# huggingface/parler-tts

Measured on NVIDIA H100. Metric: audio codec tokens/sec (all codebooks), higher is better.
Workload: dtype bf16

## Files before the change

### parler_tts_b200/csrc/attn_core.cuh

```cuda
#pragma once
#include "common.cuh"
#include "kernels.h"

namespace ptts {

constexpr int ATT_THREADS = 128;
constexpr int ATT_WARPS = 4;
constexpr int HD = PTTS_HEAD_DIM;

template <typename Sync>
__device__ __forceinline__ float block_reduce(float v, float* sh, bool is_max, int tid, Sync sync) {
  const int warp = tid >> 5, lane = tid & 31;
  v = is_max ? warp_max(v) : warp_sum(v);
  sync();
  if (lane == 0) sh[warp] = v;
  sync();
  float r = sh[0];
#pragma unroll
  for (int w = 1; w < ATT_WARPS; w++) r = is_max ? fmaxf(r, sh[w]) : r + sh[w];
  return r;
}

template <typename T>
__device__ __forceinline__ float rope_elem(float x, float x_pair, int d, const T* cos_row, const T* sin_row) {
// ... 11 lines not shown
  float* red = sm + HD;
  float* sh = red + ATT_WARPS * HD;
  float* sc = sh + 8;
  const int warp = tid >> 5, lane = tid & 31;
  const int rep = p.nh / p.nkv;
  int past = p.past_len;
  if (p.past_from_ctrl) past = p.prefix + p.ctrl->cur_len - 1;

  T* kc = reinterpret_cast<T*>(p.kcache) + (size_t)b * p.kv_b_stride + (size_t)kvh * p.kv_h_stride;
  T* vc = reinterpret_cast<T*>(p.vcache) + (size_t)b * p.kv_b_stride + (size_t)kvh * p.kv_h_stride;

  if (!p.cross) {
    const int d = tid & 63;
    const bool is_v = tid >= 64;
    for (int j = 0; j < p.q_len && j < q_hi; j++) {
      const size_t r = (size_t)b * p.q_len + j;
      const int pos = past + j;
      if (!is_v) {
        const T* src = reinterpret_cast<const T*>(p.knew) + r * p.ldkv + p.k_col0 + kvh * HD;
        float x = DT<T>::to_f(src[d]);
        if (p.rope) {
          const float xp = DT<T>::to_f(src[d < HD / 2 ? d + HD / 2 : d - HD / 2]);
          x = rope_elem<T>(x, xp, d, rope_cos + (size_t)pos * HD, rope_sin + (size_t)pos * HD);
        }
        kc[(size_t)pos * p.kv_t_stride + kv_swz(pos, d)] = DT<T>::from_f(x);
      } else {
        const T* src = reinterpret_cast<const T*>(p.vnew) + r * p.ldkv + p.v_col0 + kvh * HD;
        vc[(size_t)pos * p.kv_t_stride + kv_swz(pos, d)] = src[d];
      }
    }
    sync();
  }

  const int grp = lane >> 3;
  const int d0 = (lane & 7) * 8;
  const int kslot = warp * 4 + grp;
  const int* km = p.key_mask ? p.key_mask + (size_t)b * p.mask_ld : nullptr;

  for (int j = q_lo; j < p.q_len && j < q_hi; j++) {
    const size_t r = (size_t)b * p.q_len + j;
    const int pos = past + j;
    const int T_keys = p.cross ? p.kv_len : pos + 1;
    for (int rr = 0; rr < rep; rr++) {
      const int h = kvh * rep + rr;
      sync();
      if (tid < HD) {
        const T* src = reinterpret_cast<const T*>(p.q) + r * p.ldq + p.q_col0 + h * HD;
        float x = DT<T>::to_f(src[tid]);
        if (p.rope) {
          const float xp = DT<T>::to_f(src[tid < HD / 2 ? tid + HD / 2 : tid - HD / 2]);
          x = rope_elem<T>(x, xp, tid, rope_cos + (size_t)pos * HD, rope_sin + (size_t)pos * HD);
        }
        qs[tid] = x;
      }
      sync();
      float qv[8];
#pragma unroll
      for (int e = 0; e < 8; e++) qv[e] = qs[d0 + e];

      float lmax = -INFINITY;
      for (int t0 = 0; t0 < T_keys; t0 += 64) {
        float kv[4][8];
        bool ok[4];
#pragma unroll
        for (int u = 0; u < 4; u++) {
          const int t = t0 + u * 16 + kslot;
          ok[u] = t < T_keys;
          if (ok[u]) load8(kc + (size_t)t * p.kv_t_stride + kv_swz(t, d0), kv[u]);
        }
#pragma unroll
        for (int u = 0; u < 4; u++) {
          const int t = t0 + u * 16 + kslot;
          float s = 0.f;
          if (ok[u]) {
#pragma unroll
            for (int e = 0; e < 8; e++) s = fmaf(qv[e], kv[u][e], s);
          }
          s += __shfl_xor_sync(0xffffffffu, s, 1);
          s += __shfl_xor_sync(0xffffffffu, s, 2);
          s += __shfl_xor_sync(0xffffffffu, s, 4);
          if (ok[u] && (lane & 7) == 0) {
            s *= p.scale;
            if (km != nullptr && t < p.mask_len && km[t] == 0) s = -INFINITY;
            sc[t] = s;
            lmax = fmaxf(lmax, s);
          }
        }
      }
      const float m = block_reduce(lmax, sh, true, tid, sync);
      float lsum = 0.f;
      for (int t = tid; t < T_keys; t += ATT_THREADS) {
        const float e = (m == -INFINITY) ? 1.0f : expf(sc[t] - m);
        sc[t] = e;
        lsum += e;
      }
      const float l = block_reduce(lsum, sh, false, tid, sync);
      float acc[8];
#pragma unroll
      for (int e = 0; e < 8; e++) acc[e] = 0.f;
      for (int t0 = 0; t0 < T_keys; t0 += 64) {
        float vv[4][8];
        float pw[4];
#pragma unroll
        for (int u = 0; u < 4; u++) {
          const int t = t0 + u * 16 + kslot;
          pw[u] = 0.f;
          if (t < T_keys) {
            load8(vc + (size_t)t * p.kv_t_stride + kv_swz(t, d0), vv[u]);
            pw[u] = DT<T>::rnd(sc[t]);
          } else {
#pragma unroll
            for (int e = 0; e < 8; e++) vv[u][e] = 0.f;
          }
        }
#pragma unroll
        for (int u = 0; u < 4; u++)
#pragma unroll
          for (int e = 0; e < 8; e++) acc[e] = fmaf(pw[u], vv[u][e], acc[e]);
      }
#pragma unroll
      for (int e = 0; e < 8; e++) {
        acc[e] += __shfl_xor_sync(0xffffffffu, acc[e], 8);
        acc[e] += __shfl_xor_sync(0xffffffffu, acc[e], 16);
      }
      if (lane < 8) {
#pragma unroll
        for (int e = 0; e < 8; e++) red[warp * HD + d0 + e] = acc[e];
      }
      sync();
      if (tid < HD) {
        float o = red[tid] + red[HD + tid] + red[2 * HD + tid] + red[3 * HD + tid];
        o = o / l;
        reinterpret_cast<T*>(p.out)[r * p.ldo + h * HD + tid] = DT<T>::from_f(o);
      }
    }
  }
}

}

namespace ptts {

__device__ __forceinline__ uint32_t att_smem_u32(const void* p) { return (uint32_t)__cvta_generic_to_shared(p); }

template <typename T> struct AttChunk { static constexpr int CH = 32; };
template <> struct AttChunk<float> { static constexpr int CH = 16; };

template <typename T, int CH = AttChunk<T>::CH>
__host__ __device__ constexpr int attn_decode_smem_per_warp() {
  return 2 * 2 * CH * HD * (int)sizeof(T) + (3 * HD) * (int)sizeof(float);
}

template <typename T, int CH = AttChunk<T>::CH>
__device__ __forceinline__ void attention_decode_item_warp(const AttnArgs& p, int b, int kvh, int pos, unsigned char* sm_warp, uint64_t* bars,
                                                           int lane, uint32_t& parity, int part = 0, int nparts = 1, float* xch = nullptr,
                                                           int pair_bar = 0) {
  constexpr int STAGE_ELEMS = CH * HD;
  T* kst = reinterpret_cast<T*>(sm_warp);
  T* vst = kst + 2 * STAGE_ELEMS;
  float* qs = reinterpret_cast<float*>(vst + 2 * STAGE_ELEMS);
  float* kn = qs + HD;
  float* vn = kn + HD;
  const T* __restrict__ rope_cos = reinterpret_cast<const T*>(p.rope_cos) + (size_t)pos * HD;
  const T* __restrict__ rope_sin = reinterpret_cast<const T*>(p.rope_sin) + (size_t)pos * HD;
  const int rep = p.nh / p.nkv;
  T* kc = reinterpret_cast<T*>(p.kcache) + (size_t)b * p.kv_b_stride + (size_t)kvh * p.kv_h_stride;
  T* vc = reinterpret_cast<T*>(p.vcache) + (size_t)b * p.kv_b_stride + (size_t)kvh * p.kv_h_stride;
  const int lo = lane, hi = lane + HD / 2;
  const int n_cached = p.cross ? p.kv_len : pos;
  const int n_chunks_all = (n_cached + CH - 1) / CH;
  const int n_chunks = (n_chunks_all > part) ? (n_chunks_all - part + nparts - 1) / nparts : 0;

  auto issue = [&](int i) {
    const int st = i & 1;
    const int t0 = (part + nparts * i) * CH;
    const int n = (n_cached - t0 < CH) ? (n_cached - t0) : CH;
    const uint32_t bar = att_smem_u32(&bars[st]);
    if (lane == 0) asm volatile("mbarrier.arrive.expect_tx.shared::cta.b64 _, [%0], %1;" ::"r"(bar), "r"((uint32_t)(2 * n * HD * sizeof(T))) : "memory");
    __syncwarp();
    if (lane < 2) {
      const T* src = (lane == 0 ? kc : vc) + (size_t)t0 * HD;
      T* dst = (lane == 0 ? kst : vst) + st * STAGE_ELEMS;
      asm volatile("cp.async.bulk.shared::cluster.global.mbarrier::complete_tx::bytes [%0], [%1], %2, [%3];"
                   ::"r"(att_smem_u32(dst)), "l"(src), "r"((uint32_t)(n * HD * sizeof(T))), "r"(bar) : "memory");
    }
  };
  auto wait_stage = [&](int st) {
    const uint32_t bar = att_smem_u32(&bars[st]);
    const uint32_t par = (parity >> st) & 1u;
    uint32_t ok, spins = 0;
    do {
      asm volatile("{\n.reg .pred p;\nmbarrier.try_wait.parity.shared::cta.b64 p, [%1], %2;\nselp.u32 %0, 1, 0, p;\n}" : "=r"(ok) : "r"(bar), "r"(par) : "memory");
      if (!ok && ++spins > (1u << 16)) { if (lane == 0) printf("ptts: attention KV mbarrier timeout (cta %d b %d kvh %d stage %d cross %d n_cached %d chunks %d par %u)\n", (int)blockIdx.x, b, kvh, st, p.cross, n_cached, n_chunks, parity); __trap(); }
    } while (!ok);
    parity ^= (1u << st);
  };

  __syncwarp();
  asm volatile("fence.proxy.async.shared::cta;" ::: "memory");
  if (n_chunks > 0) issue(0);
  if (n_chunks > 1) issue(1);

  const T* q_first = reinterpret_cast<const T*>(p.q) + (size_t)b * p.ldq + p.q_col0 + (size_t)(kvh * rep) * HD;
  const float qf0 = DT<T>::to_f(q_first[lo]), qf1 = DT<T>::to_f(q_first[hi]);
  if (!p.cross && part == 0) {
    const T* ksrc = reinterpret_cast<const T*>(p.knew) + (size_t)b * p.ldkv + p.k_col0 + kvh * HD;
    const T* vsrc = reinterpret_cast<const T*>(p.vnew) + (size_t)b * p.ldkv + p.v_col0 + kvh * HD;
    float x0 = DT<T>::to_f(ksrc[lo]), x1 = DT<T>::to_f(ksrc[hi]);
    if (p.rope) {
      const float y0 = rope_elem<T>(x0, x1, lo, rope_cos, rope_sin);
      const float y1 = rope_elem<T>(x1, x0, hi, rope_cos, rope_sin);
      x0 = y0; x1 = y1;
    }
    const T v0 = vsrc[lo], v1 = vsrc[hi];
    kc[(size_t)pos * p.kv_t_stride + kv_swz(pos, lo)] = DT<T>::from_f(x0);
    kc[(size_t)pos * p.kv_t_stride + kv_swz(pos, hi)] = DT<T>::from_f(x1);
    vc[(size_t)pos * p.kv_t_stride + kv_swz(pos, lo)] = v0;
    vc[(size_t)pos * p.kv_t_stride + kv_swz(pos, hi)] = v1;
    kn[lo] = DT<T>::rnd(x0); kn[hi] = DT<T>::rnd(x1);
    vn[lo] = DT<T>::to_f(v0); vn[hi] = DT<T>::to_f(v1);
  }
  const int grp = lane >> 3, d0 = (lane & 7) * 8;
  const int* km = p.key_mask ? p.key_mask + (size_t)b * p.mask_ld : nullptr;

  for (int rr = 0; rr < rep; rr++) {
    const int h = kvh * rep + rr;
    {
      const T* qsrc = reinterpret_cast<const T*>(p.q) + (size_t)b * p.ldq + p.q_col0 + h * HD;
      float x0 = (rr == 0) ? qf0 : DT<T>::to_f(qsrc[lo]), x1 = (rr == 0) ? qf1 : DT<T>::to_f(qsrc[hi]);
      if (p.rope) {
        const float y0 = rope_elem<T>(x0, x1, lo, rope_cos, rope_sin);
        const float y1 = rope_elem<T>(x1, x0, hi, rope_cos, rope_sin);
        x0 = y0; x1 = y1;
      }
      __syncwarp();
      qs[lo] = x0; qs[hi] = x1;
      __syncwarp();
    }
    float qv[8];
#pragma unroll
    for (int e = 0; e < 8; e++) qv[e] = qs[d0 + e];
    float m_run = -INFINITY, l_run = 0.f;
    float acc[8];
#pragma unroll
    for (int e = 0; e < 8; e++) acc[e] = 0.f;

    auto process = [&](const T* kb, const T* vb, uint32_t mword, int n) {
      constexpr int PER = CH / 4;
      float sloc[PER];
#pragma unroll
      for (int u = 0; u < PER; u++) {
        const int r = u * 4 + grp, rc = r < n ? r : n - 1;
        float kf[8];
        load8(kb + rc * HD + kv_swz(rc, d0), kf);
        float s = 0.f;
#pragma unroll
        for (int e = 0; e < 8; e++) s = fmaf(qv[e], kf[e], s);
        sloc[u] = s;
      }
#pragma unroll
      for (int u = 0; u < PER; u++) sloc[u] += __shfl_xor_sync(0xffffffffu, sloc[u], 1);
#pragma unroll
      for (int u = 0; u < PER; u++) sloc[u] += __shfl_xor_sync(0xffffffffu, sloc[u], 2);
#pragma unroll
      for (int u = 0; u < PER; u++) sloc[u] += __shfl_xor_sync(0xffffffffu, sloc[u], 4);
      float cmax = -INFINITY;
#pragma unroll
      for (int u = 0; u < PER; u++) {
        const int r = u * 4 + grp;
        sloc[u] = (r < n && ((mword >> r) & 1u)) ? sloc[u] * p.scale : -INFINITY;
        cmax = fmaxf(cmax, sloc[u]);
      }
      cmax = warp_max(cmax);
      const float m_new = fmaxf(m_run, cmax);
      if (m_new == -INFINITY) return;
      const float corr = (m_run == -INFINITY) ? 0.f : expf(m_run - m_new);
      l_run *= corr;
#pragma unroll
      for (int e = 0; e < 8; e++) acc[e] *= corr;
      float lsum = 0.f;
#pragma unroll
      for (int u = 0; u < PER; u++) {
        const int r = u * 4 + grp, rc = r < n ? r : n - 1;
        const float pe = expf(sloc[u] - m_new);
        lsum += pe;
        const float pw = DT<T>::rnd(pe);
        float vf[8];
        load8(vb + rc * HD + kv_swz(rc, d0), vf);
#pragma unroll
        for (int e = 0; e < 8; e++) acc[e] = fmaf(pw, vf[e], acc[e]);
      }
      lsum += __shfl_xor_sync(0xffffffffu, lsum, 8);
      lsum += __shfl_xor_sync(0xffffffffu, lsum, 16);
      l_run += lsum;
      m_run = m_new;
    };
    auto mask_bits = [&](int t0) -> int {
      const int t = t0 + lane;
      return (km != nullptr && lane < CH && t < p.mask_len && t < n_cached) ? km[t] : 1;
    };

    if (rr > 0) {
      __syncwarp();
      asm volatile("fence.proxy.async.shared::cta;" ::: "memory");
      if (n_chunks > 0) issue(0);
      if (n_chunks > 1) issue(1);
    }
    for (int c = 0; c < n_chunks; c++) {
      const int st = c & 1;
      const int t0 = (part + nparts * c) * CH;
      const int n = (n_cached - t0 < CH) ? (n_cached - t0) : CH;
      const int mk = mask_bits(t0);
      wait_stage(st);
      process(kst + st * STAGE_ELEMS, vst + st * STAGE_ELEMS, __ballot_sync(0xffffffffu, mk != 0), n);
      if (c + 2 < n_chunks) {
        __syncwarp();
        asm volatile("fence.proxy.async.shared::cta;" ::: "memory");
        issue(c + 2);
      }
    }
    if (!p.cross && part == 0) {
      __syncwarp();
      float s = 0.f;
      if (grp == 0) {
#pragma unroll
        for (int e = 0; e < 8; e++) s = fmaf(qv[e], kn[d0 + e], s);
      }
      s += __shfl_xor_sync(0xffffffffu, s, 1);
      s += __shfl_xor_sync(0xffffffffu, s, 2);
      s += __shfl_xor_sync(0xffffffffu, s, 4);
      s = __shfl_sync(0xffffffffu, s, 0) * p.scale;
      if (km != nullptr && pos < p.mask_len && km[pos] == 0) s = -INFINITY;
      const float m_new = fmaxf(m_run, s);
      if (m_new != -INFINITY) {
        const float corr = (m_run == -INFINITY) ? 0.f : expf(m_run - m_new);
        const float pe = (s == -INFINITY) ? 0.f : expf(s - m_new);
        const float pw = DT<T>::rnd(pe);
        l_run = l_run * corr + pe;
#pragma unroll
        for (int e = 0; e < 8; e++) acc[e] = acc[e] * corr + ((grp == 0) ? pw * vn[d0 + e] : 0.f);
        m_run = m_new;
      }
    }
#pragma unroll
    for (int e = 0; e < 8; e++) {
      acc[e] += __shfl_xor_sync(0xffffffffu, acc[e], 8);
      acc[e] += __shfl_xor_sync(0xffffffffu, acc[e], 16);
    }
    if (nparts == 2) {
      if (part == 1) {
        if (lane < 8) {
#pragma unroll
          for (int e = 0; e < 8; e++) xch[d0 + e] = acc[e];
        }
        if (lane == 0) { xch[HD] = m_run; xch[HD + 1] = l_run; }
      }
      asm volatile("bar.sync %0, 64;" ::"r"(pair_bar) : "memory");
      if (part == 0) {
        const float m1 = xch[HD], l1 = xch[HD + 1];
        const float mm = fmaxf(m_run, m1);
        const float c0 = (m_run == -INFINITY) ? 0.f : expf(m_run - mm);
        const float c1 = (m1 == -INFINITY) ? 0.f : expf(m1 - mm);
        l_run = l_run * c0 + l1 * c1;
        if (lane < 8) {
#pragma unroll
          for (int e = 0; e < 8; e++) acc[e] = acc[e] * c0 + xch[d0 + e] * c1;
        }
      }
      asm volatile("bar.sync %0, 64;" ::"r"(pair_bar) : "memory");
    }
    if (lane < 8 && part == 0) {
      float o[8];
      const float inv = (l_run > 0.f) ? 1.0f / l_run : 0.f;
#pragma unroll
      for (int e = 0; e < 8; e++) o[e] = acc[e] * inv;
      store8(reinterpret_cast<T*>(p.out) + (size_t)b * p.ldo + h * HD + d0, o);
    }
  }
}

__device__ __forceinline__ void att_ldsm4(uint32_t (&r)[4], uint32_t addr) {
  asm volatile("ldmatrix.sync.aligned.m8n8.x4.shared.b16 {%0,%1,%2,%3}, [%4];" : "=r"(r[0]), "=r"(r[1]), "=r"(r[2]), "=r"(r[3]) : "r"(addr));
}
__device__ __forceinline__ void att_ldsm4_t(uint32_t (&r)[4], uint32_t addr) {
  asm volatile("ldmatrix.sync.aligned.m8n8.x4.trans.shared.b16 {%0,%1,%2,%3}, [%4];" : "=r"(r[0]), "=r"(r[1]), "=r"(r[2]), "=r"(r[3]) : "r"(addr));
}
__device__ __forceinline__ void att_mma(float (&d)[4], uint32_t a0, uint32_t a1, uint32_t a2, uint32_t a3, uint32_t b0, uint32_t b1) {
  asm volatile("mma.sync.aligned.m16n8k16.row.col.f32.bf16.bf16.f32 {%0,%1,%2,%3}, {%4,%5,%6,%7}, {%8,%9}, {%0,%1,%2,%3};"
               : "+f"(d[0]), "+f"(d[1]), "+f"(d[2]), "+f"(d[3]) : "r"(a0), "r"(a1), "r"(a2), "r"(a3), "r"(b0), "r"(b1));
}
__device__ __forceinline__ uint32_t att_pack(float lo, float hi) {
  const __nv_bfloat162 v = __floats2bfloat162_rn(lo, hi);
  return *reinterpret_cast<const uint32_t*>(&v);
}

__device__ __forceinline__ float att_ex2(float x) {
  float y;
  asm("ex2.approx.ftz.f32 %0, %1;" : "=f"(y) : "f"(x));
  return y;
}

__device__ __forceinline__ void att_bulk_kv(uint32_t dst, const void* src, uint32_t bytes, uint32_t bar, bool stream) {
  if (stream) {
    uint64_t pol;
    asm volatile("createpolicy.fractional.L2::evict_first.b64 %0, 1.0;" : "=l"(pol));
    asm volatile("cp.async.bulk.shared::cluster.global.mbarrier::complete_tx::bytes.L2::cache_hint [%0], [%1], %2, [%3], %4;"
                 ::"r"(dst), "l"(src), "r"(bytes), "r"(bar), "l"(pol) : "memory");
  } else {
    asm volatile("cp.async.bulk.shared::cluster.global.mbarrier::complete_tx::bytes [%0], [%1], %2, [%3];"
                 ::"r"(dst), "l"(src), "r"(bytes), "r"(bar) : "memory");
  }
}

constexpr int ATT_TC_CH = 32;
constexpr int ATT_TC_STAGE_BYTES = 2 * ATT_TC_CH * HD * 2;

struct TcItem {
  const bf16* q;
  const bf16* knew;
  const bf16* vnew;
  bf16* kc;
  bf16* vc;
  const int* km;
  int mask_len;
  int n_cached;
  int pos;
  int cross;
  int rope;
  const bf16* rope_cos;
  const bf16* rope_sin;
  float scale;
  bf16* out;
};

__device__ __forceinline__ void attention_tc_issue_first(const TcItem& p, unsigned char* ring0, uint64_t* bars, int lane,
                                                         int part, int nparts, bool stream = false) {
  constexpr int CH = ATT_TC_CH;
  const int n_cached = p.n_cached;
  const int t0 = part * CH;
  if (t0 >= n_cached) return;
  const int n = (n_cached - t0 < CH) ? (n_cached - t0) : CH;
  const bf16* kc = p.kc;
  const bf16* vc = p.vc;
  __syncwarp();
  const uint32_t bar = att_smem_u32(&bars[0]);
  if (lane == 0) asm volatile("mbarrier.arrive.expect_tx.shared::cta.b64 _, [%0], %1;" ::"r"(bar), "r"((uint32_t)(2 * n * HD * 2)) : "memory");
  __syncwarp();
  if (lane < 2) {
    const bf16* src = (lane == 0 ? kc : vc) + (size_t)t0 * HD;
    bf16* dst = reinterpret_cast<bf16*>(ring0) + (lane == 0 ? 0 : CH * HD);
    att_bulk_kv(att_smem_u32(dst), src, (uint32_t)(n * HD * 2), bar, stream);
  }
}

__device__ __forceinline__ void attention_decode_item_warp_tc(const TcItem& p, unsigned char* ring0, unsigned char* ring1, float* fbuf,
                                                              uint64_t* bars, int lane, uint32_t& parity, int part, int nparts, float* xch, int pair_bar,
                                                              long long* prof = nullptr, bool pre_issued = false, bool stream = false) {
  constexpr int CH = ATT_TC_CH;
  constexpr int NTS = CH / 8;
  constexpr int KPV = CH / 16;
  float* qs = fbuf;
  float* kn = qs + HD;
  float* vn = kn + HD;
  const int pos = p.pos;
  const bf16* __restrict__ rope_cos = p.rope ? p.rope_cos + (size_t)pos * HD : nullptr;
  const bf16* __restrict__ rope_sin = p.rope ? p.rope_sin + (size_t)pos * HD : nullptr;
  bf16* kc = p.kc;
// ... 228 lines not shown
```

### parler_tts_b200/csrc/step2.cu

```cuda
#include "attn_core.cuh"
#include "common.cuh"
#include "kernels.h"
#include "ln_stats.cuh"
#include "sample_core.cuh"
#include "step.h"
#include <type_traits>

#include <cstdlib>

namespace ptts {
namespace cl {

constexpr int C = 2;
constexpr int V = 8;
constexpr int THREADS = 256;
constexpr int ROWS = 32;
constexpr int HROWS = 8;
constexpr int ATT_SMEM = attn_decode_smem_per_warp<bf16>();
constexpr int PROF_STRIDE = 16;
constexpr int QMAX = 6;
constexpr int OFF_STATS = 256, OFF_PART = 512, OFF_RES = 2560, OFF_CVEC = 3584;
constexpr int HDR = 5632;
constexpr int WB_BYTES = 65536;
constexpr int R_OFF = HDR + 2 * WB_BYTES;
constexpr int R_BYTES = 92160;
constexpr int R_PASS0 = 65536;
constexpr int QKV_OFF = R_BYTES - 2048;
constexpr int SMEM_BYTES = R_OFF + R_BYTES;
static_assert(SMEM_BYTES + 1024 <= 227 * 1024, "cluster step kernel shared memory");
static_assert(ROWS * (1024 / 2 + 8) * 2 <= V * (256 + ROWS * 34 * 4) && 2 * V * (256 + ROWS * 34 * 4) <= R_BYTES, "fc1 plan");
static_assert(2 * V * C * (32 + 4 * 96 * 4) <= R_PASS0 && R_PASS0 + V * QMAX * 32 * 16 <= QKV_OFF, "QKV plan");
static_assert(5 * ATT_SMEM <= QKV_OFF && 3 * ATT_SMEM <= WB_BYTES && 16384 + 4 * 128 * 4 <= WB_BYTES, "attention plan");
static_assert(ROWS * (4096 / 4 + 8) * 2 + V * (256 + ROWS * 8 * 4) <= R_BYTES, "fc2 plan");

__device__ __forceinline__ uint32_t s32(const void* p) { return (uint32_t)__cvta_generic_to_shared(p); }
__device__ __forceinline__ void mbar_init(uint64_t* bar, uint32_t count) { asm volatile("mbarrier.init.shared::cta.b64 [%0], %1;" ::"r"(s32(bar)), "r"(count)); }
__device__ __forceinline__ void mbar_expect_tx(uint64_t* bar, uint32_t bytes) {
  asm volatile("mbarrier.arrive.expect_tx.shared::cta.b64 _, [%0], %1;" ::"r"(s32(bar)), "r"(bytes) : "memory");
}
__device__ __forceinline__ void mbar_wait(uint64_t* bar, uint32_t parity, int what) {
  uint32_t ok, spins = 0;
  do {
    asm volatile("{\n.reg .pred p;\nmbarrier.try_wait.parity.acquire.cluster.shared::cta.b64 p, [%1], %2;\nselp.u32 %0, 1, 0, p;\n}"
                 : "=r"(ok) : "r"(s32(bar)), "r"(parity) : "memory");
    if (!ok && ++spins > (1u << 22)) { printf("ptts: cluster step mbarrier timeout (cta %d, barrier kind %d)\n", (int)blockIdx.x, what); __trap(); }
  } while (!ok);
}
__device__ __forceinline__ void bulk_g2s(void* dst_smem, const void* src, uint32_t bytes, uint64_t* bar) {
  asm volatile("cp.async.bulk.shared::cluster.global.mbarrier::complete_tx::bytes [%0], [%1], %2, [%3];"
               ::"r"(s32(dst_smem)), "l"(src), "r"(bytes), "r"(s32(bar)) : "memory");
}
__device__ __forceinline__ uint64_t l2_evict_first_policy() {
  uint64_t pol;
  asm volatile("createpolicy.fractional.L2::evict_first.b64 %0, 1.0;" : "=l"(pol));
  return pol;
}
__device__ __forceinline__ void bulk_g2s_stream(void* dst_smem, const void* src, uint32_t bytes, uint64_t* bar) {
  asm volatile("cp.async.bulk.shared::cluster.global.mbarrier::complete_tx::bytes.L2::cache_hint [%0], [%1], %2, [%3], %4;"
               ::"r"(s32(dst_smem)), "l"(src), "r"(bytes), "r"(s32(bar)), "l"(l2_evict_first_policy()) : "memory");
}
__device__ __forceinline__ void bulk_s2peer(uint32_t dst_cluster_addr, const void* src_smem, uint32_t bytes, uint32_t bar_cluster_addr) {
  asm volatile("cp.async.bulk.shared::cluster.shared::cta.mbarrier::complete_tx::bytes [%0], [%1], %2, [%3];"
               ::"r"(dst_cluster_addr), "r"(s32(src_smem)), "r"(bytes), "r"(bar_cluster_addr) : "memory");
}
__device__ __forceinline__ uint32_t mapa(uint32_t addr, uint32_t rank) { uint32_t r; asm volatile("mapa.shared::cluster.u32 %0, %1, %2;" : "=r"(r) : "r"(addr), "r"(rank)); return r; }
__device__ __forceinline__ uint32_t cluster_rank() { uint32_t r; asm volatile("mov.u32 %0, %%cluster_ctarank;" : "=r"(r)); return r; }
__device__ __forceinline__ void cluster_arrive() { asm volatile("barrier.cluster.arrive.release.aligned;" ::: "memory"); }
__device__ __forceinline__ void cluster_wait() { asm volatile("barrier.cluster.wait.acquire.aligned;" ::: "memory"); }
__device__ __forceinline__ void cluster_arrive_reuse(bool release) {
  if (release) asm volatile("barrier.cluster.arrive.release.aligned;" ::: "memory");
  else asm volatile("barrier.cluster.arrive.relaxed.aligned;" ::: "memory");
}
__device__ __forceinline__ void fence_proxy_async_smem() { asm volatile("fence.proxy.async.shared::cta;" ::: "memory"); }
__device__ __forceinline__ void l2_prefetch(const void* p, uint32_t bytes, bool on = true) {
  if (!on) return;
  const char* c = reinterpret_cast<const char*>(p);
  while (bytes > 0) {
    const uint32_t n = bytes > 32768u ? 32768u : bytes;
    asm volatile("cp.async.bulk.prefetch.L2.global [%0], %1;" ::"l"(c), "r"(n) : "memory");
    c += n;
    bytes -= n;
  }
}
__device__ __forceinline__ unsigned ld_relaxed(const unsigned* p) { unsigned v; asm volatile("ld.relaxed.gpu.global.u32 %0, [%1];" : "=r"(v) : "l"(p) : "memory"); return v; }
__device__ __forceinline__ void red_release_add(unsigned* p, unsigned v) { asm volatile("red.release.gpu.global.add.u32 [%0], %1;" ::"l"(p), "r"(v) : "memory"); }
__device__ __forceinline__ void ldsm4(uint32_t (&r)[4], const void* smem_ptr) {
  asm volatile("ldmatrix.sync.aligned.m8n8.x4.shared.b16 {%0,%1,%2,%3}, [%4];" : "=r"(r[0]), "=r"(r[1]), "=r"(r[2]), "=r"(r[3]) : "r"(s32(smem_ptr)));
}
__device__ __forceinline__ void prof_mark(long long* prof, int slot) { if (prof != nullptr && threadIdx.x == 0) prof[slot] = clock64(); }

template <typename Post, typename Side>
__device__ __forceinline__ unsigned grid_sync(unsigned* ctr, unsigned target, int ph, Post post, Side side, bool acq_fence = true) {
  target += gridDim.x;
  asm volatile("fence.proxy.async.global;" ::: "memory");
  __syncthreads();
  if (threadIdx.x == 0) {
    red_release_add(ctr, 1u);
    unsigned spins = 0;
    while (ld_relaxed(ctr) < target) {
      if (++spins > (1u << 24)) { printf("ptts: cluster step grid barrier timeout (cta %d target %u seen %u phase %d)\n", (int)blockIdx.x, target, ld_relaxed(ctr), ph); __trap(); }
    }
    if (acq_fence) asm volatile("fence.acq_rel.gpu;" ::: "memory");
    post();
  } else if (threadIdx.x == 32) {
    side();
  }
  __syncthreads();
  return target;
}

__host__ __device__ __forceinline__ int kslice(int kt) { return (kt & 7) >> 2; }
__host__ __device__ __forceinline__ int klocal(int kt) { return ((kt >> 3) << 2) | (kt & 3); }
__host__ __device__ __forceinline__ int kglobal(int rank, int lk) { return ((lk >> 2) << 3) | (rank << 2) | (lk & 3); }

template <int QN, int MT, bool STATS, bool ACC = false>
__device__ __forceinline__ void mma_slice(float (&out)[2][6][4], RowStatFrag& rst, const bf16* xs, int apitch, const uint4* wb, int KT, int kt0,
                                          int kt_end, int lrow, int lcol) {
  float acc[MT][QN][4];
#pragma unroll
  for (int a = 0; a < MT; a++)
#pragma unroll
    for (int j = 0; j < QN; j++)
#pragma unroll
      for (int e = 0; e < 4; e++) acc[a][j][e] = ACC ? out[a][j][e] : 0.f;
  for (int kt = kt0; kt < kt_end; kt += 4) {
    uint32_t a[MT][2][4];
#pragma unroll
    for (int mt = 0; mt < MT; mt++)
#pragma unroll
      for (int j = 0; j < 2; j++) ldsm4(a[mt][j], xs + (size_t)(mt * 16 + lrow) * apitch + kt * 32 + j * 16 + lcol);
    if (STATS) {
#pragma unroll
      for (int mt = 0; mt < MT; mt++) { row_stat_mma(rst, mt, a[mt][0]); row_stat_mma(rst, mt, a[mt][1]); }
    }
#pragma unroll
    for (int j = 0; j < QN; j++) {
      const uint4 w = wb[((size_t)j * KT + kt) * 32];
#pragma unroll
      for (int mt = 0; mt < MT; mt++) {
        mma_bf16_16816(acc[mt][j], a[mt][0], w.x, w.y);
        mma_bf16_16816(acc[mt][j], a[mt][1], w.z, w.w);
      }
    }
  }
#pragma unroll
  for (int mt = 0; mt < MT; mt++)
#pragma unroll
    for (int j = 0; j < QN; j++)
#pragma unroll
      for (int e = 0; e < 4; e++) out[mt][j][e] = acc[mt][j][e];
}

enum { PH_QKV = 0, PH_O = 1, PH_QC = 2, PH_OC = 3, PH_FC1 = 4, PH_FC2 = 5 };
constexpr int JOBS_PER_LAYER = 9;
constexpr int QKV_JOBS = 4;

__device__ __forceinline__ bool weight_job(const StepParams& p, int j, int cta, int rank, const char*& src, uint32_t& bytes) {
  const int nl = JOBS_PER_LAYER * p.L;
  if (j < nl) {
    const int l = j / JOBS_PER_LAYER, jl = j - JOBS_PER_LAYER * l;
    const int ph = jl < QKV_JOBS ? 0 : jl - (QKV_JOBS - 1);
    const int64_t idx = (ph == PH_QKV || ph == PH_QC) ? (int64_t)(cta >> 3) * C + rank : (int64_t)cta;
    const int64_t sz = p.cp_slice[ph];
    bytes = (uint32_t)(ph == PH_QKV ? sz / QKV_JOBS : sz);
    src = p.blob + p.layer0 + p.layer_stride * l + p.cp[ph] + idx * sz + (ph == PH_QKV ? jl * (sz / QKV_JOBS) : 0);
    return true;
  }
  const int task = cta + (int)gridDim.x * (j - nl);
  const int ntasks = p.K * p.V / 32;
  if (task >= ntasks) return false;
  bytes = (uint32_t)(4 * p.H * 16);
  src = p.blob + p.heads + (int64_t)task * bytes;
  return true;
}

template <int ITEMS>
__global__ void __launch_bounds__(THREADS, 1) decode_step_cluster_kernel(const __grid_constant__ StepParams p) {
  extern __shared__ __align__(128) unsigned char smem[];
  Ctrl* ctrl = p.sa.ctrl;
  if (p.prof != nullptr && blockIdx.x == 0 && threadIdx.x == 0) p.prof[(size_t)(6 * p.L + 2) * PROF_STRIDE + 3] = clock64();
  if (ctrl->active == 0) return;
  int cur_len = ctrl->cur_len;
  const unsigned gen = (unsigned)ctrl->launch_gen;
  int pos = p.P + cur_len - 1;
  const int tid = threadIdx.x, warp = tid >> 5, lane = tid & 31;
// ... 77 lines not shown
    const int lk = klocal(n >> 5), kq = KsF >> 5;
    return (size_t)(2 * kslice(n >> 5) + lk / kq) * h_slice_elems + (lk % kq) * 32 + (n & 31);
  };
  const int xo_slice = kslice(cta >> 2), xo_col = klocal(cta >> 2) * 32 + (cta & 3) * 8;

  {
    const bf16* tables = reinterpret_cast<const bf16*>(blob + p.embed);
    const bf16* postab = p.rope ? nullptr : reinterpret_cast<const bf16*>(blob + p.pos);
    const int row = tid >> 3, f = tid & 7, n = cta * 8 + f;
    float v = 0.f;
    if (row < B) {
#pragma unroll 1
      for (int k0 = 0; k0 < p.K; k0 += 8) {
        float ev[8];
#pragma unroll
        for (int k = 0; k < 8; k++)
          if (k0 + k < p.K) ev[k] = __bfloat162float(tables[((size_t)(k0 + k) * (p.V + 1) + p.sa.cur_ids[row * p.K + k0 + k]) * H + n]);
#pragma unroll
        for (int k = 0; k < 8; k++)
          if (k0 + k < p.K) v = (k0 + k == 0) ? ev[k] : DT<bf16>::rnd(v + ev[k]);
      }
      if (postab != nullptr) v = DT<bf16>::rnd(v + __bfloat162float(postab[(size_t)pos * H + n]));
    }
    res_s[row * 8 + f] = v;
    x_img[(size_t)xo_slice * x_slice_elems + row * pitch + xo_col + f] = __float2bfloat16_rn(v);
  }
  prof_mark(prof, 6);
  auto request_slice = [&](const bf16* img_slice, uint32_t bytes) {
    fence_proxy_async_smem();
    mbar_expect_tx(abar, bytes);
    bulk_g2s(Rg, img_slice, bytes, abar);
  };
  auto slice_of = [&](int sub, const bf16*& img, uint32_t& bytes) {
    if (sub == PH_QKV || sub == PH_QC) { img = x_img + (size_t)rank * x_slice_elems + (size_t)(HROWS * rblk) * pitch; bytes = (uint32_t)(HROWS * pitch * 2); }
    else if (sub == PH_O || sub == PH_OC) { img = a_img + (size_t)rank * x_slice_elems; bytes = (uint32_t)(x_slice_elems * 2); }
    else if (sub == PH_FC1) { img = x_img + (size_t)rank * x_slice_elems; bytes = (uint32_t)(x_slice_elems * 2); }
    else { img = h_img + (size_t)(2 * rank) * h_slice_elems; bytes = (uint32_t)(h_slice_elems * 2); }
  };
  {
    const bf16* nimg; uint32_t nbytes;
    slice_of(PH_QKV, nimg, nbytes);
    bar_target = grid_sync(bar_ctr, bar_target, -1, [&]() { request_slice(nimg, nbytes); }, []() {}, acq);
  }
  prof_mark(prof, 7);

  const int lrow = (lane & 7) + ((lane >> 3) & 1) * 8, lcol = (lane >> 4) * 8;
  const int g = lane >> 2, t4 = lane & 3;
  const int n_phases = 6 * p.L;

  const int att_row = HROWS * rblk + 4 * rank + (warp >> 1);
  const int att_slice = kslice(2 * head), att_col = klocal(2 * head) * 32;

#pragma unroll 1
  for (int ph = 0; ph < n_phases; ph++) {
    const int l = ph / 6, sub = ph - 6 * l;
    prof = prof0 ? prof0 + (size_t)(ph + 1) * PROF_STRIDE : nullptr;
    prof_mark(prof, 0);
    const char* lb = blob + p.layer0 + p.layer_stride * l;
    const bool rowpart = (sub == PH_QKV || sub == PH_QC);
    const bool has_ln = (sub == PH_QKV || sub == PH_QC || sub == PH_FC1);
    const int q = (sub == PH_QKV) ? 6 : (sub == PH_QC ? 2 : (sub == PH_FC1 ? qe : 1));
    const int Nc = 4 * q * 8;
    const int KT = (sub == PH_FC2 ? KsF : Ks) >> 5;
    const int apitch = (sub == PH_FC2) ? pitchF : pitch;
    const int act_bytes = (rowpart ? HROWS : ROWS) * apitch * 2;
    const int RS = (q == 1) ? 8 : 8 * q + 2;
    const int blk = rowpart ? 32 + 4 * 16 * q * 4 : 256 + ROWS * RS * 4;
    const int wsend = rowpart ? C * blk : blk;
    const int j0 = JOBS_PER_LAYER * l + (sub == 0 ? 0 : sub + QKV_JOBS - 1);
    const int njobs = sub == 0 ? QKV_JOBS : 1;

    float cv1 = 0.f, cv2 = 0.f;
    if (has_ln) {
      const float* c1; int ntot;
      if (sub == PH_QKV) { c1 = reinterpret_cast<const float*>(lb + p.c_qkv); ntot = p.qkv_rows; }
      else if (sub == PH_QC) { c1 = reinterpret_cast<const float*>(lb + p.c_qc); ntot = H; }
      else { c1 = reinterpret_cast<const float*>(lb + p.c_fc1); ntot = F; }
      const int nown = rowpart ? Nc : 8 * q;
      if (tid < nown) {
        int n;
        if (sub == PH_QKV) n = (tid >> 6) * (p.nh * HD) + head * HD + (tid & 63);
        else if (sub == PH_QC) n = head * HD + tid;
        else n = cta * 8 * q + tid;
        cv1 = c1[n];
        cv2 = c1[ntot + n];
      }
    }

    auto wait_job = [&](int j) {
      mbar_wait(&wbar[j & 1], (par_w >> (j & 1)) & 1u, 1);
      par_w ^= 1u << (j & 1);
    };
    auto ring = [&](int j) { return reinterpret_cast<const uint4*>(smem + HDR + (j & 1) * WB_BYTES) + lane; };
    wait_job(j0);
    if (sub == PH_QKV) wait_job(j0 + 1);
    mbar_wait(abar, par_a, 0);
    par_a ^= 1u;
    prof_mark(prof, 1);
    float acc[2][QMAX][4];
    float4* const pass0 = reinterpret_cast<float4*>(Rg + R_PASS0) + (size_t)warp * QMAX * 32 + lane;
    RowStatFrag rst;
    row_stat_zero(rst);
    {
      const bf16* xs = reinterpret_cast<const bf16*>(Rg);
      if (rowpart) {
        auto head_pass = [&](auto pass_tag) {
          constexpr int P = decltype(pass_tag)::value;
          const int u = 2 * P + dgrp;
          float t[2][QMAX][4];
          if (sub == PH_QKV) mma_slice<6, 1, P == 0>(t, rst, xs, apitch, ring(j0 + u), KT, e4, KT, lrow & 7, lcol);
          else mma_slice<2, 1, P == 0>(t, rst, xs, apitch, ring(j0) + (size_t)(2 * u) * KT * 32, KT, e4, KT, lrow & 7, lcol);
#pragma unroll
          for (int j = 0; j < QMAX; j++)
            if (j < q) {
              if (P == 0) pass0[j * 32] = make_float4(t[0][j][0], t[0][j][1], t[0][j][2], t[0][j][3]);
              else {
#pragma unroll
                for (int e = 0; e < 4; e++) acc[0][j][e] = t[0][j][e];
              }
            }
        };
        head_pass(std::integral_constant<int, 0>{});
        if (sub == PH_QKV) {
          __syncthreads();
          if (tid == 0) { issue_weight_job(j0 + 2); issue_weight_job(j0 + 3); }
          wait_job(j0 + 2);
          wait_job(j0 + 3);
        }
        head_pass(std::integral_constant<int, 1>{});
      } else if (sub == PH_FC2) {
        auto quarter = [&](auto qq_tag) {
          constexpr int QQ = decltype(qq_tag)::value;
          const uint4* wq = ring(j0) + (size_t)dgrp * 2 * KT * 32 + (size_t)QQ * KT * 32;
          mma_slice<1, 2, false, QQ == 1>(acc, rst, xs, apitch, wq, 2 * KT, (e4 - QQ * KT) & 3, KT, lrow, lcol);
        };
        quarter(std::integral_constant<int, 0>{});
        __syncthreads();
        if (tid == 0) request_slice(h_img + (size_t)(2 * rank + 1) * h_slice_elems, (uint32_t)(h_slice_elems * 2));
        mbar_wait(abar, par_a, 0);
        par_a ^= 1u;
        quarter(std::integral_constant<int, 1>{});
      } else {
        const uint4* wb = ring(j0) + (size_t)(dgrp * q) * KT * 32;
        if (sub == PH_FC1) {
          if (q == 4) mma_slice<4, 2, true>(acc, rst, xs, apitch, wb, KT, e4, KT, lrow, lcol);
          else if (q == 2) mma_slice<2, 2, true>(acc, rst, xs, apitch, wb, KT, e4, KT, lrow, lcol);
          else mma_slice<1, 2, true>(acc, rst, xs, apitch, wb, KT, e4, KT, lrow, lcol);
        } else mma_slice<1, 2, false>(acc, rst, xs, apitch, wb, KT, e4, KT, lrow, lcol);
      }
    }
    prof_mark(prof, 2);
    if (has_ln && tid < (rowpart ? Nc : 8 * q)) { cvec[tid] = cv1; cvec[256 + tid] = cv2; }
    __syncthreads();
    if (lane == 0 && (pf_on || pf_kv)) {
      for (int i = 0; i < njobs; i++) prefetch_weight_job_part(j0 + i + JOBS_PER_LAYER, warp);
      if (sub == PH_QKV && warp == 2 && l + 1 < p.L) {
        const int64_t c_bytes = p.c_fc1 + (int64_t)2 * F * 4 - p.c_qkv;
        const uint32_t share = (uint32_t)(((c_bytes / (int)gridDim.x) + 15) & ~15);
        const int64_t o = (int64_t)cta * share;
        if (pf_on && o < c_bytes) l2_prefetch(lb + p.layer_stride + p.c_qkv + o, (uint32_t)(c_bytes - o < share ? c_bytes - o : share));
      }
      if (sub == PH_O && l + 1 < p.L) prefetch_kv_part(l + 1, false, warp);
      if (sub == PH_OC && l + 1 < p.L) prefetch_kv_part(l + 1, true, warp);
    }
    prof_mark(prof, 12);
    cluster_wait();
    prof_mark(prof, 13);

    const int nslots = rowpart ? V * C : V;
    unsigned char* send = Rg;
    const int send_end = V * wsend;
    unsigned char* recv = Rg + (((send_end > act_bytes ? send_end : act_bytes) + 127) & ~127);
    if (tid == 0) mbar_expect_tx(xbar, (uint32_t)(nslots * blk));
    {
      unsigned char* mine = send + (size_t)warp * wsend;
      const bool merged = rowpart && !(p.dbg & 1024);
      if (!rowpart) {
        float* bp = reinterpret_cast<float*>(mine + 256);
#pragma unroll
        for (int mt = 0; mt < 2; mt++)
#pragma unroll
          for (int j = 0; j < QMAX; j++) {
            if (j < q) {
              float* base = bp + (size_t)(mt * 16 + g) * RS + j * 8 + 2 * t4;
              *reinterpret_cast<float2*>(base) = make_float2(acc[mt][j][0], acc[mt][j][1]);
              *reinterpret_cast<float2*>(base + 8 * RS) = make_float2(acc[mt][j][2], acc[mt][j][3]);
            }
          }
        if (has_ln) {
          float* st = reinterpret_cast<float*>(mine);
#pragma unroll
          for (int mt = 0; mt < 2; mt++) {
            const int r0 = mt * 16 + g;
            if (t4 == 0) { st[2 * r0] = rst.s1[mt][0]; st[2 * (r0 + 8)] = rst.s1[mt][2]; }
            if (t4 == (g >> 1)) {
              st[2 * r0 + 1] = (g & 1) ? rst.sq[mt][0][1] : rst.sq[mt][0][0];
              st[2 * (r0 + 8) + 1] = (g & 1) ? rst.sq[mt][1][3] : rst.sq[mt][1][2];
            }
          }
        }
      } else {
        const int qc = 16 * q;
        unsigned char* blk_d = merged ? send + ((size_t)(g >> 2) * V + warp) * blk : mine + (size_t)(g >> 2) * blk;
        float* bp = reinterpret_cast<float*>(blk_d + 32) + (g & 3) * qc + 2 * t4;
#pragma unroll
        for (int P = 0; P < 2; P++)
#pragma unroll
          for (int j = 0; j < QMAX; j++)
            if (j < q) *reinterpret_cast<float2*>(bp + P * 8 * q + j * 8) = P == 0 ? make_float2(pass0[j * 32].x, pass0[j * 32].y)
                                                                                   : make_float2(acc[0][j][0], acc[0][j][1]);
        float* st = reinterpret_cast<float*>(blk_d) + (g & 3) * 2;
        if (t4 == 0) st[0] = rst.s1[0][0];
        if (t4 == (g >> 1)) st[1] = (g & 1) ? rst.sq[0][0][1] : rst.sq[0][0][0];
      }
      __syncwarp();
      prof_mark(prof, 14);
      if (!rowpart) {
        if (lane == 0) {
          fence_proxy_async_smem();
          bulk_s2peer(mapa(s32(recv + (size_t)(4 * rank + e4) * blk), (uint32_t)dgrp), mine, (uint32_t)blk, mapa(s32(xbar), (uint32_t)dgrp));
        }
      } else if (merged) {
        __syncthreads();
        if (warp < C && lane == 0) {
          fence_proxy_async_smem();
          bulk_s2peer(mapa(s32(recv + (size_t)(8 * rank) * blk), (uint32_t)warp), send + (size_t)warp * V * blk, (uint32_t)(V * blk), mapa(s32(xbar), (uint32_t)warp));
        }
      } else if (lane < C) {
        fence_proxy_async_smem();
        bulk_s2peer(mapa(s32(recv + (size_t)(8 * rank + warp) * blk), (uint32_t)lane), mine + (size_t)lane * blk, (uint32_t)blk, mapa(s32(xbar), (uint32_t)lane));
      }
    }
    if (warp == 1 && lane == 0 && !rowpart) issue_weight_job(j0 + 2);
    if (warp == 1 && lane == 0 && sub == PH_QKV) issue_weight_job(j0 + QKV_JOBS);
    prof_mark(prof, 15);
    mbar_wait(xbar, par_x, 2);
    par_x ^= 1u;
    prof_mark(prof, 3);

    if (!rowpart) {
      const int row = tid >> 3, f0 = tid & 7;
      float ln_mean = 0.f, ln_rstd = 0.f;
      if (has_ln) {
        float S1 = 0.f, S2 = 0.f;
#pragma unroll
        for (int v = 0; v < V; v++) { const float2 x = *reinterpret_cast<const float2*>(recv + (size_t)v * blk + row * 8); S1 += x.x; S2 += x.y; }
        ln_mean = S1 / (float)H;
        ln_rstd = rsqrtf(fmaxf(S2 / (float)H - ln_mean * ln_mean, 0.f) + p.eps);
      }
      if (row < B && sub == PH_FC1 && q == 4) {
        const int f = 4 * f0;
        float v[4] = {0.f, 0.f, 0.f, 0.f};
#pragma unroll
        for (int sv = 0; sv < V; sv++) {
          const float* bp = reinterpret_cast<const float*>(recv + (size_t)sv * blk + 256) + row * RS + f;
          const float2 a = *reinterpret_cast<const float2*>(bp), b2 = *reinterpret_cast<const float2*>(bp + 2);
          v[0] += a.x; v[1] += a.y; v[2] += b2.x; v[3] += b2.y;
        }
#pragma unroll
        for (int e = 0; e < 4; e++) v[e] = apply_act(DT<bf16>::rnd(ln_rstd * (v[e] - ln_mean * cvec[f + e]) + cvec[256 + f + e]), p.act);
        uint2 pk;
        pk.x = att_pack(v[0], v[1]); pk.y = att_pack(v[2], v[3]);
        *reinterpret_cast<uint2*>(h_img + h_offset(cta * 32 + f) + row * pitchF) = pk;
      } else if (row < B) {
        for (int i = 0; i < q; i++) {
          const int f = f0 + 8 * i;
          float v = 0.f;
#pragma unroll
          for (int sv = 0; sv < V; sv++) v += reinterpret_cast<const float*>(recv + (size_t)sv * blk + 256)[row * RS + f];
          if (sub == PH_FC1) {
            v = ln_rstd * (v - ln_mean * cvec[f]) + cvec[256 + f];
            v = apply_act(DT<bf16>::rnd(v), p.act);
            h_img[h_offset(cta * 8 * q + f) + row * pitchF] = __float2bfloat16_rn(v);
          } else {
            v = DT<bf16>::rnd(res_s[row * 8 + f] + DT<bf16>::rnd(v));
            res_s[row * 8 + f] = v;
            x_img[(size_t)xo_slice * x_slice_elems + row * pitch + xo_col + f] = __float2bfloat16_rn(v);
          }
        }
      }
    } else {
      bf16* qkv_s = reinterpret_cast<bf16*>(Rg + QKV_OFF);
      auto gather = [&](auto jw_tag) {
        constexpr int JW = decltype(jw_tag)::value, NC = 4 * JW, QCW = 2 * JW;
        for (int idx = tid; idx < 4 * NC; idx += THREADS) {
          const int r4 = idx / NC, col = idx - r4 * NC;
          const int u = col / JW, cw = (u >> 1) * JW + (col - u * JW);
          float S1 = 0.f, S2 = 0.f;
#pragma unroll
          for (int e = 0; e < V; e++) {
            const float2 x = *reinterpret_cast<const float2*>(recv + (size_t)(8 * (e >> 2) + 2 * (e & 3)) * blk + r4 * 8);
            S1 += x.x; S2 += x.y;
          }
          const float ln_mean = S1 / (float)H;
          const float ln_rstd = rsqrtf(fmaxf(S2 / (float)H - ln_mean * ln_mean, 0.f) + p.eps);
          float v = 0.f;
#pragma unroll
          for (int e = 0; e < V; e++)
            v += reinterpret_cast<const float*>(recv + (size_t)(8 * (e >> 2) + 2 * (e & 3) + (u & 1)) * blk + 32)[r4 * QCW + cw];
          v = ln_rstd * (v - ln_mean * cvec[col]) + cvec[256 + col];
          qkv_s[idx] = __float2bfloat16_rn(v);
        }
      };
      if (sub == PH_QKV) gather(std::integral_constant<int, 48>{}); else gather(std::integral_constant<int, 16>{});
      static_assert(HD == 64, "QKV: 2 x 2 units of 6 n-tiles (q|k|v of a head), q_cross: 2 x 2 units of 2 n-tiles");
    }
    prof_mark(prof, 4);
    __syncthreads();
    cluster_arrive_reuse((p.dbg & 64) != 0);
    if (rowpart) {
      cluster_wait();
      cluster_arrive();
    }

    if (rowpart) {
      if (att_row < B) {
        AttnArgs att{};
        att.ctrl = nullptr; att.B = B; att.nh = p.nh; att.nkv = p.nh; att.q_len = 1;
        att.past_from_ctrl = 0; att.past_len = pos; att.prefix = p.P;
        att.rope = p.rope; att.rope_cos = blob + p.rope_cos; att.rope_sin = blob + p.rope_sin; att.scale = p.scale;
        const bf16* qkv_s = reinterpret_cast<const bf16*>(Rg + QKV_OFF);
        const int row_base = HROWS * rblk + 4 * rank;
        const bf16* qbase = qkv_s - (size_t)row_base * Nc - (size_t)head * HD;
        att.q = qbase; att.ldq = Nc; att.q_col0 = 0;
        att.ldo = pitch;
        att.out = a_img + (size_t)att_slice * x_slice_elems + att_col - (size_t)head * HD;
        if (sub == PH_QKV) {
          att.knew = qbase; att.vnew = qbase; att.ldkv = Nc; att.k_col0 = HD; att.v_col0 = 2 * HD;
          char* kc = p.self_kv + p.self_layer_stride * l;
          att.kcache = kc; att.vcache = kc + (size_t)B * p.nh * p.Tmax * HD * 2;
          att.kv_b_stride = (int64_t)p.nh * p.Tmax * HD; att.kv_h_stride = (int64_t)p.Tmax * HD; att.kv_t_stride = HD;
          att.key_mask = p.prompt_mask; att.mask_len = p.P; att.mask_ld = p.P;
          att.cross = 0; att.kv_len = 0; att.kv_capacity = p.Tmax;
        } else {
          att.knew = nullptr; att.vnew = nullptr;
          char* ck = p.cross_kv + p.cross_layer_stride * l;
          att.kcache = ck; att.vcache = ck + (size_t)B * p.nh * p.S * HD * 2;
          att.kv_b_stride = (int64_t)p.nh * p.S * HD; att.kv_h_stride = (int64_t)p.S * HD; att.kv_t_stride = HD;
          att.key_mask = p.enc_mask; att.mask_len = p.S; att.mask_ld = p.S;
          att.cross = 1; att.kv_len = p.S; att.kv_capacity = p.S;
        }
        unsigned char* wb0 = smem + HDR;
        unsigned char* held = wb0 + ((sub == PH_QKV ? j0 + 1 : j0) & 1) * WB_BYTES;
        unsigned char* other = wb0 + ((sub == PH_QKV ? j0 : j0 + 1) & 1) * WB_BYTES;
        unsigned char* region = warp < 5 ? Rg + (size_t)warp * ATT_SMEM : held + (size_t)(warp - 5) * ATT_SMEM;
        float* xr = reinterpret_cast<float*>(other + 16384) + (warp >> 1) * 128;
        attention_decode_item_warp<bf16>(att, att_row, head, pos, region, attbars + 2 * warp, lane, att_parity, warp & 1, 2, xr, (warp >> 1) + 1);
      }
      prof_mark(prof, 5);
      __syncthreads();
      if (tid == 32) {
        fence_proxy_async_smem();
        issue_weight_job(sub == PH_QKV ? j0 + QKV_JOBS + 1 : j0 + 2);
      }
    }
    prof_mark(prof, 6);
    if (p.prof != nullptr && l == p.L / 2 && tid == 0) {
      unsigned long long ns;
      asm volatile("mov.u64 %0, %%globaltimer;" : "=l"(ns));
      p.prof[(size_t)(n_phases + 4) * PROF_STRIDE + sub * (int)gridDim.x + cta] = (long long)ns;
    }

    const bool last = (ph + 1 == n_phases);
    const bf16* nimg; uint32_t nbytes;
    if (last) { nimg = x_img; nbytes = (uint32_t)(C * x_slice_elems * 2); }
    else slice_of((sub + 1) % 6, nimg, nbytes);
    bar_target = grid_sync(bar_ctr, bar_target, ph, [&]() { request_slice(nimg, nbytes); }, []() {}, acq);
    prof_mark(prof, 7);
  }
  cluster_wait();

  prof = prof0 ? prof0 + (size_t)(n_phases + 1) * PROF_STRIDE : nullptr;
  prof_mark(prof, 0);
  {
    const int ntasks = p.K * p.V / 32;
    const float* c1 = reinterpret_cast<const float*>(blob + p.c_heads);
    const float* c2 = c1 + p.K * p.V;
    if (lane == 0) {
      for (int j = 0; j < JOBS_PER_LAYER; j++) prefetch_weight_job_part(j, warp);
    }
    mbar_wait(abar, par_a, 3);
    par_a ^= 1u;
    const bf16* xs = reinterpret_cast<const bf16*>(Rg);
    const int KTH = H >> 5;
    auto ktile = [&](int kt) { return xs + (size_t)kslice(kt) * x_slice_elems + klocal(kt) * 32; };
    {
      RowStatFrag rst;
      row_stat_zero(rst);
      for (int kt = warp; kt < KTH; kt += 8) {
        const bf16* sl = ktile(kt);
#pragma unroll
        for (int mt = 0; mt < 2; mt++)
#pragma unroll
          for (int j = 0; j < 2; j++) {
            uint32_t a[4];
            ldsm4(a, sl + (size_t)(mt * 16 + lrow) * pitch + j * 16 + lcol);
            row_stat_mma(rst, mt, a);
          }
      }
      row_stat_store(rst, part, warp, lane);
      __syncthreads();
      row_stat_finalize(part, H, ROWS, p.eps, stats);
      __syncthreads();
    }
    prof_mark(prof, 1);
    constexpr int HRS = 40;
    int job = JOBS_PER_LAYER * p.L;
    for (int task = cta; task < ntasks; task += (int)gridDim.x, job++) {
      mbar_wait(&wbar[job & 1], (par_w >> (job & 1)) & 1u, 4);
      par_w ^= 1u << (job & 1);
      float acc[2][4][4];
#pragma unroll
      for (int a = 0; a < 2; a++)
#pragma unroll
        for (int j = 0; j < 4; j++)
#pragma unroll
          for (int e = 0; e < 4; e++) acc[a][j][e] = 0.f;
      unsigned char* wbuf = smem + HDR + (job & 1) * WB_BYTES;
      const uint4* wb = reinterpret_cast<const uint4*>(wbuf) + lane;
      for (int kt = warp; kt < KTH; kt += 8) {
        const bf16* sl = ktile(kt);
        uint32_t a[2][2][4];
#pragma unroll
        for (int mt = 0; mt < 2; mt++)
#pragma unroll
          for (int j = 0; j < 2; j++) ldsm4(a[mt][j], sl + (size_t)(mt * 16 + lrow) * pitch + j * 16 + lcol);
#pragma unroll
        for (int j = 0; j < 4; j++) {
          const uint4 w = wb[((size_t)j * KTH + kt) * 32];
#pragma unroll
          for (int mt = 0; mt < 2; mt++) {
            mma_bf16_16816(acc[mt][j], a[mt][0], w.x, w.y);
            mma_bf16_16816(acc[mt][j], a[mt][1], w.z, w.w);
          }
        }
      }
      __syncthreads();
      float* red = reinterpret_cast<float*>(wbuf);
#pragma unroll
      for (int mt = 0; mt < 2; mt++)
#pragma unroll
        for (int j = 0; j < 4; j++) {
          float* base = red + ((size_t)warp * 32 + mt * 16 + g) * HRS + j * 8 + 2 * t4;
          *reinterpret_cast<float2*>(base) = make_float2(acc[mt][j][0], acc[mt][j][1]);
          *reinterpret_cast<float2*>(base + 8 * HRS) = make_float2(acc[mt][j][2], acc[mt][j][3]);
        }
      __syncthreads();
      {
        const int er = tid >> 3, ec = tid & 7;
        if (er < B) {
          const float mean = stats[2 * er], rstd = stats[2 * er + 1];
#pragma unroll
          for (int j = 0; j < 4; j++) {
            const int cidx = j * 8 + ec, n = task * 32 + cidx;
            float v = 0.f;
#pragma unroll
            for (int w = 0; w < 8; w++) v += red[((size_t)w * 32 + er) * HRS + cidx];
            p.logits[(size_t)er * p.K * p.V + n] = DT<bf16>::rnd(rstd * (v - mean * c1[n]) + c2[n]);
          }
        }
      }
      __syncthreads();
      if (tid == 32) {
        fence_proxy_async_smem();
        issue_weight_job(job + 2);
      }
    }
  }
  prof_mark(prof, 6);
  bar_target = grid_sync(bar_ctr, bar_target, n_phases, []() {}, []() {});
  prof = prof0 ? prof0 + (size_t)(n_phases + 2) * PROF_STRIDE : nullptr;
  prof_mark(prof, 0);
  if (p.do_sample_phase) {
    const ptts_gen_params gp = *p.sa.gen;
    const int BK = B * p.K;
    for (int pass = (p.dbg & 128) ? 0 : 1; pass < 2; pass++) {
      sample_all_rows_cta<ITEMS>(p.sa, gp, cta, (int)gridDim.x, BK, cur_len);
      prof_mark(prof, pass == 0 ? 4 : 1);
    }
    bar_target = grid_sync(bar_ctr, bar_target, n_phases + 1, [&]() {
      const int tot = *reinterpret_cast<volatile int*>(&ctrl->n_unfinished);
      s_next_active = (tot - unfinished_prev > 0) ? 1 : 0;
      unfinished_prev = tot;
    }, []() {});
    prof_mark(prof, 2);
  }
  bool go_on = false;
  if (p.do_sample_phase) {
    const int act = s_next_active;
    if (cta == 0 && tid == 0) {
      ctrl->cur_len = cur_len + 1;
      ctrl->active = act;
      ctrl->steps_run += 1;
    }
    go_on = act != 0;
    cur_len += 1;
  }
  if (!go_on) break;
  }
  if (cta == 0 && tid == 0) {
// ... 89 lines not shown
```

Before: 212,300.

## Pre-issue first KV chunk TMA load before cluster exchange in decode attention

```diff
diff --git a/parler_tts_b200/csrc/attn_core.cuh b/parler_tts_b200/csrc/attn_core.cuh
--- a/parler_tts_b200/csrc/attn_core.cuh
+++ b/parler_tts_b200/csrc/attn_core.cuh
@@ -187,13 +187,35 @@
 }
 
 template <typename T, int CH = AttChunk<T>::CH>
+__device__ __forceinline__ void attention_decode_issue_first(const T* kc, const T* vc, int n_cached, unsigned char* ring0, uint64_t* bars,
+                                                             int lane, int part) {
+  const int t0 = part * CH;
+  if (t0 >= n_cached) return;
+  const int n = (n_cached - t0 < CH) ? (n_cached - t0) : CH;
+  const uint32_t bar = att_smem_u32(&bars[0]);
+  __syncwarp();
+  if (lane == 0) asm volatile("mbarrier.arrive.expect_tx.shared::cta.b64 _, [%0], %1;" ::"r"(bar), "r"((uint32_t)(2 * n * HD * sizeof(T))) : "memory");
+  __syncwarp();
+  if (lane < 2) {
+    const T* src = (lane == 0 ? kc : vc) + (size_t)t0 * HD;
+    T* dst = reinterpret_cast<T*>(ring0) + (lane == 0 ? 0 : CH * HD);
+    asm volatile("cp.async.bulk.shared::cluster.global.mbarrier::complete_tx::bytes [%0], [%1], %2, [%3];"
+                 ::"r"(att_smem_u32(dst)), "l"(src), "r"((uint32_t)(n * HD * sizeof(T))), "r"(bar) : "memory");
+  }
+}
+
+template <typename T, int CH = AttChunk<T>::CH>
 __device__ __forceinline__ void attention_decode_item_warp(const AttnArgs& p, int b, int kvh, int pos, unsigned char* sm_warp, uint64_t* bars,
                                                            int lane, uint32_t& parity, int part = 0, int nparts = 1, float* xch = nullptr,
-                                                           int pair_bar = 0) {
+                                                           int pair_bar = 0, unsigned char* ring0 = nullptr, unsigned char* ring1 = nullptr,
+                                                           float* fbuf = nullptr, bool pre_issued = false) {
   constexpr int STAGE_ELEMS = CH * HD;
-  T* kst = reinterpret_cast<T*>(sm_warp);
-  T* vst = kst + 2 * STAGE_ELEMS;
-  float* qs = reinterpret_cast<float*>(vst + 2 * STAGE_ELEMS);
+  const bool apart = ring0 != nullptr;
+  T* const kst0 = apart ? reinterpret_cast<T*>(ring0) : reinterpret_cast<T*>(sm_warp);
+  T* const kst1 = apart ? reinterpret_cast<T*>(ring1) : kst0 + STAGE_ELEMS;
+  T* const vst0 = apart ? kst0 + STAGE_ELEMS : kst0 + 2 * STAGE_ELEMS;
+  T* const vst1 = apart ? kst1 + STAGE_ELEMS : vst0 + STAGE_ELEMS;
+  float* qs = apart ? fbuf : reinterpret_cast<float*>(vst1 + STAGE_ELEMS);
   float* kn = qs + HD;
   float* vn = kn + HD;
   const T* __restrict__ rope_cos = reinterpret_cast<const T*>(p.rope_cos) + (size_t)pos * HD;
@@ -215,7 +237,7 @@
     __syncwarp();
     if (lane < 2) {
       const T* src = (lane == 0 ? kc : vc) + (size_t)t0 * HD;
-      T* dst = (lane == 0 ? kst : vst) + st * STAGE_ELEMS;
+      T* dst = lane == 0 ? (st ? kst1 : kst0) : (st ? vst1 : vst0);
       asm volatile("cp.async.bulk.shared::cluster.global.mbarrier::complete_tx::bytes [%0], [%1], %2, [%3];"
                    ::"r"(att_smem_u32(dst)), "l"(src), "r"((uint32_t)(n * HD * sizeof(T))), "r"(bar) : "memory");
     }
@@ -233,7 +255,7 @@
 
   __syncwarp();
   asm volatile("fence.proxy.async.shared::cta;" ::: "memory");
-  if (n_chunks > 0) issue(0);
+  if (!pre_issued && n_chunks > 0) issue(0);
   if (n_chunks > 1) issue(1);
 
   const T* q_first = reinterpret_cast<const T*>(p.q) + (size_t)b * p.ldq + p.q_col0 + (size_t)(kvh * rep) * HD;
@@ -347,7 +369,7 @@
       const int n = (n_cached - t0 < CH) ? (n_cached - t0) : CH;
       const int mk = mask_bits(t0);
       wait_stage(st);
-      process(kst + st * STAGE_ELEMS, vst + st * STAGE_ELEMS, __ballot_sync(0xffffffffu, mk != 0), n);
+      process(st ? kst1 : kst0, st ? vst1 : vst0, __ballot_sync(0xffffffffu, mk != 0), n);
       if (c + 2 < n_chunks) {
         __syncwarp();
         asm volatile("fence.proxy.async.shared::cta;" ::: "memory");
diff --git a/parler_tts_b200/csrc/step2.cu b/parler_tts_b200/csrc/step2.cu
--- a/parler_tts_b200/csrc/step2.cu
+++ b/parler_tts_b200/csrc/step2.cu
@@ -16,7 +16,8 @@
 constexpr int THREADS = 256;
 constexpr int ROWS = 32;
 constexpr int HROWS = 8;
-constexpr int ATT_SMEM = attn_decode_smem_per_warp<bf16>();
+constexpr int ATT_STAGE = 2 * 32 * HD * 2;
+constexpr int ATT_R_BYTES = ATT_STAGE + 3 * HD * 4;
 constexpr int PROF_STRIDE = 16;
 constexpr int QMAX = 6;
 constexpr int OFF_STATS = 256, OFF_PART = 512, OFF_RES = 2560, OFF_CVEC = 3584;
@@ -30,7 +31,8 @@
 static_assert(SMEM_BYTES + 1024 <= 227 * 1024, "cluster step kernel shared memory");
 static_assert(ROWS * (1024 / 2 + 8) * 2 <= V * (256 + ROWS * 34 * 4) && 2 * V * (256 + ROWS * 34 * 4) <= R_BYTES, "fc1 plan");
 static_assert(2 * V * C * (32 + 4 * 96 * 4) <= R_PASS0 && R_PASS0 + V * QMAX * 32 * 16 <= QKV_OFF, "QKV plan");
-static_assert(5 * ATT_SMEM <= QKV_OFF && 3 * ATT_SMEM <= WB_BYTES && 16384 + 4 * 128 * 4 <= WB_BYTES, "attention plan");
+static_assert(8 * ATT_R_BYTES <= QKV_OFF && 8 * ATT_STAGE <= WB_BYTES && 16384 + 4 * 128 * 4 <= WB_BYTES, "attention plan");
+static_assert(AttChunk<bf16>::CH == 32, "ATT_STAGE: 32 keys per stage");
 static_assert(ROWS * (4096 / 4 + 8) * 2 + V * (256 + ROWS * 8 * 4) <= R_BYTES, "fc2 plan");
 
 __device__ __forceinline__ uint32_t s32(const void* p) { return (uint32_t)__cvta_generic_to_shared(p); }
@@ -414,6 +416,15 @@
     prof_mark(prof, 2);
     if (has_ln && tid < (rowpart ? Nc : 8 * q)) { cvec[tid] = cv1; cvec[256 + tid] = cv2; }
     __syncthreads();
+    unsigned char* const att_held = smem + HDR + ((sub == PH_QKV ? j0 + 1 : j0) & 1) * WB_BYTES;
+    if (rowpart && att_row < B) {
+      const bool self = sub == PH_QKV;
+      const int T = self ? p.Tmax : p.S;
+      const bf16* kc = reinterpret_cast<const bf16*>(self ? p.self_kv + p.self_layer_stride * l : p.cross_kv + p.cross_layer_stride * l) +
+                       ((size_t)att_row * p.nh + head) * T * HD;
+      attention_decode_issue_first<bf16>(kc, kc + (size_t)B * p.nh * T * HD, self ? pos : p.S, att_held + (size_t)warp * ATT_STAGE, attbars + 2 * warp,
+                                         lane, warp & 1);
+    }
     if (lane == 0 && (pf_on || pf_kv)) {
       for (int i = 0; i < njobs; i++) prefetch_weight_job_part(j0 + i + JOBS_PER_LAYER, warp);
       if (sub == PH_QKV && warp == 2 && l + 1 < p.L) {
@@ -602,12 +613,11 @@
           att.key_mask = p.enc_mask; att.mask_len = p.S; att.mask_ld = p.S;
           att.cross = 1; att.kv_len = p.S; att.kv_capacity = p.S;
         }
-        unsigned char* wb0 = smem + HDR;
-        unsigned char* held = wb0 + ((sub == PH_QKV ? j0 + 1 : j0) & 1) * WB_BYTES;
-        unsigned char* other = wb0 + ((sub == PH_QKV ? j0 : j0 + 1) & 1) * WB_BYTES;
-        unsigned char* region = warp < 5 ? Rg + (size_t)warp * ATT_SMEM : held + (size_t)(warp - 5) * ATT_SMEM;
+        unsigned char* other = smem + HDR + ((sub == PH_QKV ? j0 : j0 + 1) & 1) * WB_BYTES;
+        unsigned char* r1 = Rg + (size_t)warp * ATT_R_BYTES;
         float* xr = reinterpret_cast<float*>(other + 16384) + (warp >> 1) * 128;
-        attention_decode_item_warp<bf16>(att, att_row, head, pos, region, attbars + 2 * warp, lane, att_parity, warp & 1, 2, xr, (warp >> 1) + 1);
+        attention_decode_item_warp<bf16>(att, att_row, head, pos, nullptr, attbars + 2 * warp, lane, att_parity, warp & 1, 2, xr, (warp >> 1) + 1,
+                                         att_held + (size_t)warp * ATT_STAGE, r1, reinterpret_cast<float*>(r1 + ATT_STAGE), true);
       }
       prof_mark(prof, 5);
       __syncthreads();
```

Measured after the change: 221,100, median of 6. +4.2%, better.
